# e-c-k-e-r/tortoise-tts

Hardware: AMD Instinct MI355X
Metric: audio-sec/wall-sec (RTF^-1), 16 AR candidates x 80 DDIM steps (higher is better)
Workload: dtype bf16; 1 GPU; configs[1]: 1 utterance/GPU, 64 text tokens, 16 AR candidates x 250 mel tokens (KV-cached decode), latent pass on 16 candidates, 80 DDIM steps with cond-free guidance at T=1088 (11.6 s audio); candidates=16, ddim_steps=80, mel_frames=1088, parallelism=single GPU, small_models=False, vocoder_in_step=False

## Files before the change

### tortoise_tts_amd/csrc/ar.hip

```cpp
#include "ttk_common.h"
#include "ttk_host.h"

using namespace ttk;

namespace {

struct ARLayer {
	float *ln1_g, *ln1_b, *ln2_g, *ln2_b;
	Mat attn, proj, fc, proj2;
};

__global__ void k_build_prefill_emb(const float* cond, int Bc, const int64_t* text, int Tt, int B, int d,
									const float* text_emb, const float* text_pos, const float* mel_emb, const float* mel_pos,
									int start_text, int stop_text, int start_mel, float* out, const int64_t* prompt = nullptr, int prompt_rows = 0, int n_in = 0) {
	const int S = Tt + 4 + n_in;
	const int64_t idx = (int64_t)blockIdx.x * blockDim.x + threadIdx.x;
	const int d4 = d / 4;
	if (idx >= (int64_t)B * S * d4) return;
	const int c = (int)(idx % d4) * 4;
	const int64_t row = idx / d4;
	const int b = (int)(row / S), s = (int)(row - (int64_t)b * S);
	float4 v;
	if (s == 0) {
		v = *(const float4*)(cond + (int64_t)(Bc == 1 ? 0 : b) * d + c);
// ... 16 lines not shown
								   int start_text, int stop_text, int start_mel, int stop_mel, float* out) {
	const int S = Tt + M + 5;
	const int64_t idx = (int64_t)blockIdx.x * blockDim.x + threadIdx.x;
	const int d4 = d / 4;
	if (idx >= (int64_t)B * S * d4) return;
	const int c = (int)(idx % d4) * 4;
	const int64_t row = idx / d4;
	const int b = (int)(row / S), s = (int)(row - (int64_t)b * S);
	float4 v;
	if (s == 0) {
		v = *(const float4*)(cond + (int64_t)b * d + c);
	} else if (s < Tt + 3) {
		const int j = s - 1;
		const int64_t tok = j == 0 ? start_text : (j == Tt + 1 ? stop_text : text[(int64_t)b * Tt + j - 1]);
		const float4 e = *(const float4*)(text_emb + tok * d + c), w = *(const float4*)(text_pos + (int64_t)j * d + c);
		v = make_float4(e.x + w.x, e.y + w.y, e.z + w.z, e.w + w.w);
	} else {
		const int j = s - (Tt + 3);
		const int64_t tok = j == 0 ? start_mel : (j == M + 1 ? stop_mel : codes[(int64_t)b * M + j - 1]);
		const float4 e = *(const float4*)(mel_emb + tok * d + c), w = *(const float4*)(mel_pos + (int64_t)j * d + c);
		v = make_float4(e.x + w.x, e.y + w.y, e.z + w.z, e.w + w.w);
	}
	*(float4*)(out + row * d + c) = v;
}

}

struct ttk_ar {
	ttk_ar_config cfg;
	int dt;
	int wdt;
	size_t es;
	Arena arena;
	std::vector<ARLayer> L;
	float *lnf_g, *lnf_b, *fn_g, *fn_b;
	Mat head;
	float *text_emb, *mel_emb, *mel_pos, *text_pos;
	void *kc, *vc;
	size_t kv_layer_stride;
	int* d_pos;
	int pos_slot = -1;
	int2* d_rowinfo;
	int lines_mode = 0;
	float *x, *qbuf;
	void *attn_out, *hbuf;
	void* x_frag = nullptr;
	int poison = 0;
	int frag_rows = 0;
	int shared_rows = 0;
	int share_prefix = 1;
	const int64_t* rng_args = nullptr; const int64_t* rng_draws = nullptr; float* rng_q = nullptr;
	int* d_health = nullptr;
	float* ring_base = nullptr; const int64_t* ring_idx = nullptr; int64_t ring_stride = 0;
	int64_t* d_ring = nullptr;
	int head_split = 1;
	int lnfold = 1;
	int lean = 1;
	float* slab; int* tickets;
	int wv_proj = 4, wv_proj2 = 8;
	int wv_ln = 4;
	int wv_head = 4;
	int hfrag = 1;
	int narrow2 = 4;
	int narrow = 4;
	int nsplit = 1;
	hipStream_t side[3] = {nullptr, nullptr, nullptr};
	hipEvent_t ev_fork = nullptr, ev_join[3] = {nullptr, nullptr, nullptr};
	WsBuf ws_x, ws_a, ws_qkv, ws_ao, ws_h;
	int B = 0, P = 0, k = 0, ready = 0;
	int Pmax = 0;
	~ttk_ar() {
		for (int i = 0; i < 3; ++i) { if (side[i]) (void)hipStreamDestroy(side[i]); if (ev_join[i]) (void)hipEventDestroy(ev_join[i]); }
		if (ev_fork) (void)hipEventDestroy(ev_fork);
		attn_pos_slot_release(pos_slot);
	}
};

static int poison_scratch(ttk_ar* h, hipStream_t s) {
	if (!h->poison) return TTK_OK;
	for (WsBuf* w : {&h->ws_x, &h->ws_a, &h->ws_qkv, &h->ws_ao, &h->ws_h})
		if (w->p) TTK_HIP(hipMemsetAsync(w->p, 0xFF, w->cap, s));
	return TTK_OK;
}

static int dense_forward(ttk_ar* h, float* x, int B, int S, bool write_kv, hipStream_t s, int kv_row0 = 0, int kv_t0 = 0) {
	const int d = h->cfg.model_dim, H = h->cfg.heads, dt = h->dt;
	const int rows = B * S;
	TTK_TRY(h->ws_a.reserve((size_t)rows * d * h->es));
	TTK_TRY(h->ws_qkv.reserve((size_t)rows * 3 * d * h->es));
	TTK_TRY(h->ws_ao.reserve((size_t)rows * d * h->es));
	TTK_TRY(h->ws_h.reserve((size_t)rows * 4 * d * h->es));
	for (int l = 0; l < h->cfg.layers; ++l) {
		const ARLayer& L = h->L[l];
		launch_layernorm(dt, x, d, rows, d, L.ln1_g, L.ln1_b, nullptr, nullptr, h->ws_a.p, d, 0, s);
		GemmParams g = {};
		g.nseg = 1; g.seg[0] = {h->ws_a.p, d, 0, 0};
		g.W = L.attn.w; g.ldw = L.attn.Kpad; g.M = rows; g.N = 3 * d; g.K = d; g.bias = L.attn.bias;
		g.C = h->ws_qkv.p; g.ldc = 3 * d;
		launch_gemm(dt, g, s);
		if (write_kv) {
			const size_t row0 = (size_t)kv_row0 * H * h->cfg.max_ctx * 64;
			char* kc = (char*)h->kc + ((size_t)l * h->kv_layer_stride + row0) * h->es;
			char* vc = (char*)h->vc + ((size_t)l * h->kv_layer_stride + row0) * h->es;
			launch_kv_scatter(dt, h->ws_qkv.p, B, S, H, kc, vc, h->cfg.max_ctx, s, kv_t0);
		}
		AttnParams a = {};
		a.qkv = h->ws_qkv.p; a.ld = 3 * d; a.q_off = 0; a.k_off = d; a.v_off = 2 * d; a.head_stride = 64;
		a.out = h->ws_ao.p; a.ldo = d; a.nb = B; a.T = S; a.H = H; a.causal = 1; a.bias = nullptr; a.scale = 0.125f;
		launch_attn_fwd(dt, a, s);
		g = {};
		g.nseg = 1; g.seg[0] = {h->ws_ao.p, d, 0, 0};
		g.W = L.proj.w; g.ldw = L.proj.Kpad; g.M = rows; g.N = d; g.K = d; g.bias = L.proj.bias;
		g.residual = x; g.ldr = d; g.C = x; g.ldc = d; g.out_f32 = 1;
		launch_gemm(dt, g, s);
		launch_layernorm(dt, x, d, rows, d, L.ln2_g, L.ln2_b, nullptr, nullptr, h->ws_a.p, d, 0, s);
		g = {};
		g.nseg = 1; g.seg[0] = {h->ws_a.p, d, 0, 0};
		g.W = L.fc.w; g.ldw = L.fc.Kpad; g.M = rows; g.N = 4 * d; g.K = d; g.bias = L.fc.bias; g.act = ACT_GELU_NEW;
		g.C = h->ws_h.p; g.ldc = 4 * d;
		launch_gemm(dt, g, s);
		g = {};
		g.nseg = 1; g.seg[0] = {h->ws_h.p, 4 * d, 0, 0};
		g.W = L.proj2.w; g.ldw = L.proj2.Kpad; g.M = rows; g.N = d; g.K = 4 * d; g.bias = L.proj2.bias;
		g.residual = x; g.ldr = d; g.C = x; g.ldc = d; g.out_f32 = 1;
		launch_gemm(dt, g, s);
	}
	return TTK_OK;
}

static void head_launch(ttk_ar* h, int B, float* logits, float* hidden_out, hipStream_t s) {
	SkinnyParams p = {};
	p.Wp = h->head.wfrag; p.N = h->cfg.number_mel_codes; p.K = h->cfg.model_dim; p.M = B; p.bias = h->head.bias;
	p.ln_count = 2; p.x = h->x; p.ldx = h->cfg.model_dim;
	p.g1 = h->lnf_g; p.b1 = h->lnf_b; p.g2 = h->fn_g; p.b2 = h->fn_b; p.ln_out = hidden_out;
	p.mode = SK_STORE_F32; p.out_f32 = logits; p.ldc = h->cfg.number_mel_codes;
	if (h->rng_q) { p.qbuf = h->rng_q; p.slab = (float*)h->rng_args; p.tickets = (int*)h->rng_draws; }
	launch_skinny(h->dt, p, h->cfg.model_dim >= 1024 ? h->wv_head : 4, s);
}

static void decode_rows(ttk_ar* h, int r0, int nrows, int gi, float* logits_out, float* hidden_out, hipStream_t s, bool bump_pos) {
	const ttk_ar_config& c = h->cfg;
	const int d = c.model_dim, H = c.heads, dt = h->dt;
	const size_t es = h->es;
	float* x = h->x + (size_t)r0 * d;
	float* qbuf = h->qbuf + (size_t)r0 * d;
	char* attn_out = (char*)h->attn_out + (size_t)r0 * d * es;
	char* hbuf = (char*)h->hbuf + (size_t)r0 * 4 * d * es;
	const size_t kv_row = (size_t)H * c.max_ctx * 64 * es;
	const int wv_small = d >= 1024 ? h->wv_ln : 4;
	const int wv_prologue = d >= 1024 ? 8 : 4;
	const bool whole = r0 == 0 && nrows == h->B;
	void* xf = whole ? h->x_frag : nullptr;
	const bool lean = h->lean && whole && h->lnfold && h->hfrag;
	for (int l = 0; l < c.layers; ++l) {
		const ARLayer& L = h->L[l];
		char* kc = (char*)h->kc + (size_t)l * h->kv_layer_stride * es + r0 * kv_row;
		char* vc = (char*)h->vc + (size_t)l * h->kv_layer_stride * es + r0 * kv_row;
		SkinnyParams p = {};
		p.Wp = L.attn.wfrag; p.w8 = L.attn.w8; p.wscale = L.attn.wscale; p.N = 3 * d; p.K = d; p.M = nrows; p.bias = L.attn.bias;
		const bool fold_qkv = h->lnfold && whole && L.attn.wfrag_fold;
		if (fold_qkv) { p.Wp = L.attn.wfrag_fold; p.w8 = 0; p.bias = L.attn.bias_fold; p.g1 = L.attn.csum; p.a = xf; p.lda = d; p.a_frag = 1; }
		else { p.ln_count = 1; p.x = x; p.ldx = d; p.g1 = L.ln1_g; p.b1 = L.ln1_b; }
		p.mode = SK_QKV; p.qbuf = qbuf; p.kcache = kc; p.vcache = vc; p.d_pos = h->d_pos; p.max_ctx = c.max_ctx; p.H = H; p.q_scale = 0.125f;
		GemvParams gq = {};
		gq.Wp = p.Wp; gq.a = xf; gq.bias = p.bias; gq.csum = p.g1; gq.qbuf = qbuf; gq.kcache = kc; gq.vcache = vc; gq.d_pos = h->d_pos;
		gq.M = nrows; gq.N = 3 * d; gq.K = d; gq.max_ctx = c.max_ctx; gq.H = H; gq.q_scale = 0.125f; gq.health = h->d_health;
		if (!(lean && fold_qkv && launch_gemv(dt, GV_QKV, gq, s))) launch_skinny(dt, p, fold_qkv ? wv_small : wv_prologue, s);
		AttnDecodeParams a = {};
		a.qbuf = qbuf; a.kcache = kc; a.vcache = vc; a.d_pos = h->d_pos; a.pos_slot_p1 = h->pos_slot + 1; a.B = nrows; a.H = H; a.max_ctx = c.max_ctx; a.ctx_hint = h->P + 2 + h->k; a.out = attn_out; a.out_frag = h->hfrag && r0 == 0 && nrows == h->B; a.shared_rows = r0 == 0 && h->share_prefix && h->nsplit == 1;
		a.row_info = h->lines_mode && r0 == 0 ? h->d_rowinfo : nullptr;
		launch_attn_decode(dt, a, s);
		p = {};
		p.Wp = L.proj.wfrag; p.w8 = L.proj.w8; p.wscale = L.proj.wscale; p.N = d; p.K = d; p.M = nrows; p.bias = L.proj.bias; p.a = attn_out; p.lda = d; p.a_frag = h->hfrag && r0 == 0 && nrows == h->B;
		p.mode = SK_RESIDUAL; p.out_f32 = x; p.ldc = d; p.narrow = h->narrow; p.out_T = h->lnfold ? xf : nullptr;
		GemvParams gp = {};
		gp.Wp = p.Wp; gp.a = attn_out; gp.bias = p.bias; gp.out_f32 = x; gp.out_T = p.out_T; gp.M = nrows; gp.N = d; gp.K = d; gp.w8 = p.w8; gp.wscale = p.wscale;
		if (!(lean && p.a_frag && h->narrow == 4 && launch_gemv(dt, GV_PROJ, gp, s))) launch_skinny(dt, p, d >= 1024 ? h->wv_proj : 4, s);
		p = {};
		p.Wp = L.fc.wfrag; p.w8 = L.fc.w8; p.wscale = L.fc.wscale; p.N = 4 * d; p.K = d; p.M = nrows; p.bias = L.fc.bias;
		const bool fold_fc = h->lnfold && whole && L.fc.wfrag_fold;
		if (fold_fc) { p.Wp = L.fc.wfrag_fold; p.w8 = 0; p.bias = L.fc.bias_fold; p.g1 = L.fc.csum; p.a = xf; p.lda = d; p.a_frag = 1; }
		else { p.ln_count = 1; p.x = x; p.ldx = d; p.g1 = L.ln2_g; p.b1 = L.ln2_b; }
		p.mode = SK_ACT_T; p.act = ACT_GELU_NEW; p.out_T = hbuf; p.out_frag = h->hfrag && r0 == 0 && nrows == h->B;
		GemvParams gf = {};
		gf.Wp = p.Wp; gf.a = xf; gf.bias = p.bias; gf.csum = p.g1; gf.out_T = hbuf; gf.M = nrows; gf.N = 4 * d; gf.K = d; gf.health = h->d_health;
		if (!(lean && fold_fc && p.out_frag && launch_gemv(dt, GV_FC, gf, s))) launch_skinny(dt, p, fold_fc ? wv_small : wv_prologue, s);
		p = {};
		p.Wp = L.proj2.wfrag; p.w8 = L.proj2.w8; p.wscale = L.proj2.wscale; p.N = d; p.K = 4 * d; p.M = nrows; p.bias = L.proj2.bias; p.a = hbuf; p.lda = 4 * d; p.a_frag = h->hfrag && r0 == 0 && nrows == h->B;
		p.mode = SK_RESIDUAL; p.out_f32 = x; p.ldc = d; p.out_T = h->lnfold ? xf : nullptr;
		p.narrow = h->narrow2;
		if (d >= 1024 && !h->narrow2) {
			p.ksplit = 4; p.slab = h->slab + (size_t)gi * (d / 16) * 4 * 4 * 256; p.tickets = h->tickets + (size_t)gi * (d / 16);
		}
		GemvParams g2 = {};
		g2.Wp = p.Wp; g2.a = hbuf; g2.bias = p.bias; g2.out_f32 = x; g2.out_T = p.out_T; g2.M = nrows; g2.N = d; g2.K = 4 * d; g2.w8 = p.w8; g2.wscale = p.wscale;
		if (!(lean && p.a_frag && h->narrow2 == 4 && launch_gemv(dt, GV_PROJ, g2, s))) launch_skinny(dt, p, d >= 1024 ? h->wv_proj2 : 4, s);
	}
	SkinnyParams p = {};
	p.Wp = h->head.wfrag; p.N = c.number_mel_codes; p.K = d; p.M = nrows; p.bias = h->head.bias;
	p.mode = SK_STORE_F32; p.out_f32 = logits_out + (size_t)r0 * c.number_mel_codes; p.ldc = c.number_mel_codes;
	if (bump_pos) p.d_pos = h->d_pos;
	if (h->rng_q) { p.qbuf = h->rng_q + (size_t)r0 * c.number_mel_codes; p.slab = (float*)h->rng_args; p.tickets = (int*)(h->rng_draws + r0); p.max_ctx = r0; }
	float* hid = hidden_out ? hidden_out + (size_t)r0 * d : nullptr;
	if (h->head_split && whole) {
		if (h->ring_base && !hid) launch_layernorm(dt, x, d, nrows, d, h->lnf_g, h->lnf_b, h->fn_g, h->fn_b, h->attn_out, d, 0, s, 1, nullptr, h->ring_idx, h->ring_stride, h->d_ring);
		else launch_layernorm(dt, x, d, nrows, d, h->lnf_g, h->lnf_b, h->fn_g, h->fn_b, h->attn_out, d, 0, s, 1, hid);
		p.a = h->attn_out; p.lda = d; p.a_frag = 1;
		GemvParams gh = {};
		gh.Wp = p.Wp; gh.a = h->attn_out; gh.bias = p.bias; gh.out_f32 = p.out_f32; gh.d_pos = p.d_pos; gh.noise = p.qbuf; gh.rng = p.slab; gh.draws = (const int64_t*)p.tickets;
		gh.M = nrows; gh.N = c.number_mel_codes; gh.K = d; gh.row0 = r0;
		if (!(lean && launch_gemv(dt, GV_HEAD, gh, s)))
			launch_skinny(dt, p, 4, s);
	} else {
		p.ln_count = 2; p.x = x; p.ldx = d;
		p.g1 = h->lnf_g; p.b1 = h->lnf_b; p.g2 = h->fn_g; p.b2 = h->fn_b; p.ln_out = hid;
		launch_skinny(dt, p, d >= 1024 ? h->wv_head : 4, s);
	}
}

extern "C" {

int ttk_ar_create(ttk_ar** out, const ttk_ar_config* cfg, const ttk_weight_view* w, int n_w) {
	TTK_REQUIRE(out && cfg && w, TTK_E_ARG, "ttk_ar_create: null argument");
	TTK_REQUIRE(cfg->model_dim % 64 == 0 && cfg->heads * 64 == cfg->model_dim, TTK_E_ARG,
				"ttk_ar_create: head_dim must be 64 (model_dim %d, heads %d)", cfg->model_dim, cfg->heads);
	TTK_REQUIRE(cfg->model_dim <= 2048, TTK_E_ARG, "ttk_ar_create: model_dim %d > 2048 unsupported", cfg->model_dim);
	TTK_REQUIRE(cfg->dtype == TTK_F32 || cfg->dtype == TTK_BF16 || cfg->dtype == TTK_F16 || cfg->dtype == TTK_FP8W, TTK_E_ARG, "ttk_ar_create: bad dtype %d", cfg->dtype);
	TTK_REQUIRE(cfg->max_batch >= 1 && cfg->max_batch <= (cfg->dtype == TTK_F32 ? 32 : 64), TTK_E_ARG,
				"ttk_ar_create: max_batch %d out of range", cfg->max_batch);
	TTK_REQUIRE(cfg->max_ctx >= 8, TTK_E_ARG, "ttk_ar_create: max_ctx %d too small", cfg->max_ctx);
	std::unique_ptr<ttk_ar> h(new ttk_ar());
	h->cfg = *cfg;
	h->wdt = cfg->dtype;
	h->dt = kernel_dtype(cfg->dtype);
	h->es = dtype_size(h->dt);
	WeightMap wm(w, n_w);
	const int d = cfg->model_dim;
	h->L.resize(cfg->layers);
	for (int l = 0; l < cfg->layers; ++l) {
		const std::string p = "gpt.h." + std::to_string(l) + ".";
		ARLayer& L = h->L[l];
		TTK_TRY(upload_f32(h->arena, wm, p + "ln_1.weight", d, &L.ln1_g));
		TTK_TRY(upload_f32(h->arena, wm, p + "ln_1.bias", d, &L.ln1_b));
		TTK_TRY(upload_f32(h->arena, wm, p + "ln_2.weight", d, &L.ln2_g));
		TTK_TRY(upload_f32(h->arena, wm, p + "ln_2.bias", d, &L.ln2_b));
		TTK_TRY(upload_mat(h->arena, wm, h->wdt, p + "attn.c_attn.weight", p + "attn.c_attn.bias", PK_KN, 3 * d, d, true, &L.attn));
		TTK_TRY(upload_mat(h->arena, wm, h->wdt, p + "attn.c_proj.weight", p + "attn.c_proj.bias", PK_KN, d, d, true, &L.proj));
		TTK_TRY(upload_mat(h->arena, wm, h->wdt, p + "mlp.c_fc.weight", p + "mlp.c_fc.bias", PK_KN, 4 * d, d, true, &L.fc));
		TTK_TRY(upload_mat(h->arena, wm, h->wdt, p + "mlp.c_proj.weight", p + "mlp.c_proj.bias", PK_KN, d, 4 * d, true, &L.proj2));
		{
			TTK_TRY(fold_layernorm(h->arena, wm, h->dt, p + "attn.c_attn.weight", p + "attn.c_attn.bias", p + "ln_1.weight", p + "ln_1.bias", &L.attn));
			TTK_TRY(fold_layernorm(h->arena, wm, h->dt, p + "mlp.c_fc.weight", p + "mlp.c_fc.bias", p + "ln_2.weight", p + "ln_2.bias", &L.fc));
		}
	}
	TTK_TRY(upload_f32(h->arena, wm, "gpt.ln_f.weight", d, &h->lnf_g));
	TTK_TRY(upload_f32(h->arena, wm, "gpt.ln_f.bias", d, &h->lnf_b));
	TTK_TRY(upload_f32(h->arena, wm, "final_norm.weight", d, &h->fn_g));
	TTK_TRY(upload_f32(h->arena, wm, "final_norm.bias", d, &h->fn_b));
	TTK_TRY(upload_mat(h->arena, wm, h->dt, "mel_head.weight", "mel_head.bias", PK_NK, cfg->number_mel_codes, d, true, &h->head));
	TTK_TRY(upload_f32(h->arena, wm, "text_embedding.weight", (int64_t)cfg->number_text_tokens_p1 * d, &h->text_emb));
	TTK_TRY(upload_f32(h->arena, wm, "mel_embedding.weight", (int64_t)cfg->number_mel_codes * d, &h->mel_emb));
	TTK_TRY(upload_f32(h->arena, wm, "mel_pos_embedding.emb.weight", (int64_t)cfg->max_mel_seq_len * d, &h->mel_pos));
	TTK_TRY(upload_f32(h->arena, wm, "text_pos_embedding.emb.weight", (int64_t)cfg->max_text_seq_len * d, &h->text_pos));
	h->kv_layer_stride = (size_t)cfg->max_batch * cfg->heads * cfg->max_ctx * 64;
	TTK_TRY(h->arena.alloc(&h->kc, h->kv_layer_stride * cfg->layers * h->es));
	TTK_TRY(h->arena.alloc(&h->vc, h->kv_layer_stride * cfg->layers * h->es));
	TTK_TRY(h->arena.alloc((void**)&h->d_pos, (size_t)(4 + 2 * cfg->max_batch) * sizeof(int)));
	h->d_rowinfo = (int2*)(h->d_pos + 4);
	h->d_health = h->d_pos + 2;
	if (hipMemset(h->d_pos, 0, (size_t)(4 + 2 * cfg->max_batch) * sizeof(int)) != hipSuccess) return TTK_E_HIP;
	{
		int* words = nullptr;
		h->pos_slot = attn_pos_slot_acquire(&words);
		if (h->pos_slot >= 0) {
			h->d_pos = words;
			if (hipMemset(h->d_pos, 0, 2 * sizeof(int)) != hipSuccess) return TTK_E_HIP;
		}
	}
	TTK_TRY(h->arena.alloc((void**)&h->d_ring, sizeof(int64_t)));
	if (hipMemset(h->d_ring, 0, sizeof(int64_t)) != hipSuccess) return TTK_E_HIP;
	TTK_TRY(h->arena.alloc((void**)&h->x, (size_t)cfg->max_batch * d * sizeof(float)));
	TTK_TRY(h->arena.alloc((void**)&h->qbuf, (size_t)cfg->max_batch * d * sizeof(float)));
	const size_t frag_rows = (size_t)16 * decode_row_tiles(cfg->max_batch);
	h->frag_rows = (int)frag_rows;
	for (int B = 1; B <= cfg->max_batch; ++B)
		if (16 * decode_row_tiles(B) > h->frag_rows) { set_error("ttk_ar_create: %d rows would request %d fragment rows, %d allocated", B, 16 * decode_row_tiles(B), h->frag_rows); return TTK_E_STATE; }
	TTK_TRY(h->arena.alloc(&h->attn_out, frag_rows * d * h->es));
	if (hipMemset(h->attn_out, 0, frag_rows * d * h->es) != hipSuccess) return TTK_E_HIP;
	TTK_TRY(h->arena.alloc(&h->hbuf, frag_rows * 4 * d * h->es));
	if (hipMemset(h->hbuf, 0, frag_rows * 4 * d * h->es) != hipSuccess) return TTK_E_HIP;
	TTK_TRY(h->arena.alloc(&h->x_frag, frag_rows * d * h->es));
	if (hipMemset(h->x_frag, 0, frag_rows * d * h->es) != hipSuccess) return TTK_E_HIP;
	TTK_TRY(h->arena.alloc((void**)&h->slab, (size_t)4 * (d / 16) * 4 * 4 * 256 * sizeof(float)));
	TTK_TRY(h->arena.alloc((void**)&h->tickets, (size_t)4 * (d / 16) * sizeof(int)));
	if (hipMemset(h->tickets, 0, (size_t)4 * (d / 16) * sizeof(int)) != hipSuccess) return TTK_E_HIP;
	{
		const char* ep = getenv("TTK_DEBUG_POISON");
		h->poison = ep && atoi(ep) != 0;
		const char* en = getenv("TTK_AR_NARROW");
		h->narrow = en ? atoi(en) : 4;
		const char* ef = getenv("TTK_AR_HFRAG");
		h->hfrag = ef ? (atoi(ef) != 0) : 1;
		const char* en2 = getenv("TTK_AR_NARROW2");
		h->narrow2 = en2 ? atoi(en2) : h->narrow;
		const char* e1 = getenv("TTK_AR_WV_PROJ");
		const char* e2 = getenv("TTK_AR_WV_PROJ2");
		if (e1 && atoi(e1) >= 4 && atoi(e1) <= 16) h->wv_proj = atoi(e1);
		if (h->dt == DT_F32) { h->wv_proj = 8; h->wv_ln = 8; h->wv_proj2 = 8; }
		if (e2 && atoi(e2) >= 4 && atoi(e2) <= 16) h->wv_proj2 = atoi(e2);
		const char* e4 = getenv("TTK_AR_WV_LN");
		if (e4 && atoi(e4) >= 4 && atoi(e4) <= 16) h->wv_ln = atoi(e4);
		const char* e3 = getenv("TTK_AR_WV_HEAD");
		if (e3 && (atoi(e3) == 4 || atoi(e3) == 8)) h->wv_head = atoi(e3);
		const char* es = getenv("TTK_AR_SHARE_PREFIX");
		h->share_prefix = es ? (atoi(es) != 0) : 1;
		const char* eh = getenv("TTK_AR_HEAD_SPLIT");
		h->head_split = eh ? (atoi(eh) != 0) : 1;
		const char* el = getenv("TTK_AR_LNFOLD");
		h->lnfold = el ? (atoi(el) != 0) : 1;
		const char* eg = getenv("TTK_AR_LEAN");
		h->lean = eg ? (atoi(eg) != 0) : 1;
		const char* e = getenv("TTK_AR_SPLIT");
		h->nsplit = e ? atoi(e) : 1;
		if (h->nsplit != 1 && h->nsplit != 2 && h->nsplit != 4) h->nsplit = 1;
		if (hipEventCreateWithFlags(&h->ev_fork, hipEventDisableTiming) != hipSuccess) return TTK_E_HIP;
		for (int i = 0; i < 3; ++i) {
			if (hipStreamCreateWithFlags(&h->side[i], hipStreamNonBlocking) != hipSuccess) return TTK_E_HIP;
			if (hipEventCreateWithFlags(&h->ev_join[i], hipEventDisableTiming) != hipSuccess) return TTK_E_HIP;
		}
	}
	hipError_t e = hipDeviceSynchronize();
	if (e != hipSuccess) { set_error("ttk_ar_create: %s", hipGetErrorString(e)); return TTK_E_HIP; }
	*out = h.release();
	return TTK_OK;
}

int ttk_ar_destroy(ttk_ar* h) {
	if (!h) return TTK_OK;
	(void)hipDeviceSynchronize();
	delete h;
	return TTK_OK;
}

static int prefill_impl(ttk_ar* h, const float* cond_latent, int Bc, const int64_t* text, int Tt, const int64_t* prompt, int prompt_rows, int n_in, int B, float* logits_out,
						void* stream, const char* who) {
	TTK_REQUIRE(h && cond_latent && text && logits_out, TTK_E_ARG, "%s: null argument", who);
	const ttk_ar_config& c = h->cfg;
	TTK_REQUIRE(B >= 1 && B <= c.max_batch, TTK_E_ARG, "%s: B=%d exceeds max_batch=%d", who, B, c.max_batch);
	TTK_REQUIRE(Bc == 1 || Bc == B, TTK_E_ARG, "%s: cond batch %d must be 1 or B=%d", who, Bc, B);
	TTK_REQUIRE(Tt >= 1 && Tt + 2 <= c.max_text_seq_len, TTK_E_ARG, "%s: %d text tokens exceed the position table (%d)", who, Tt, c.max_text_seq_len - 2);
	TTK_REQUIRE(n_in == 0 || (prompt && (prompt_rows == 1 || prompt_rows == B)), TTK_E_ARG, "%s: %d prompt tokens need 1 or B=%d prompt rows (got %d)", who, n_in, B, prompt_rows);
	TTK_REQUIRE(n_in >= 0 && n_in + 2 < c.max_mel_seq_len, TTK_E_ARG, "%s: %d prompt tokens exceed the mel position table (%d)", who, n_in, c.max_mel_seq_len);
	const int S = Tt + 4 + n_in, d = c.model_dim;
	TTK_REQUIRE(S + 1 <= c.max_ctx, TTK_E_ARG, "%s: prefix of %d rows does not fit max_ctx=%d", who, S, c.max_ctx);
	hipStream_t s = (hipStream_t)stream;
	const bool shared = Bc == 1 && B > 1 && h->share_prefix && h->nsplit == 1 && (n_in == 0 || prompt_rows == 1);
	const int Bp = shared ? 1 : B;
	TTK_TRY(h->ws_x.reserve((size_t)Bp * S * d * sizeof(float)));
	float* x = (float*)h->ws_x.p;
	const int64_t total = (int64_t)Bp * S * (d / 4);
	hipLaunchKernelGGL(k_build_prefill_emb, dim3((unsigned)((total + 255) / 256)), dim3(256), 0, s, cond_latent, Bc, text, Tt, Bp, d,
					   h->text_emb, h->text_pos, h->mel_emb, h->mel_pos, c.start_text_token, c.stop_text_token, c.start_mel_token, x, prompt, prompt_rows, n_in);
	TTK_TRY(dense_forward(h, x, Bp, S, true, s));
	launch_copy_rows(x + (size_t)(S - 1) * d, shared ? 0 : (int64_t)S * d, h->x, d, B, d, s);
	head_launch(h, B, logits_out, nullptr, s);
	launch_set_int(h->d_pos, S, s);
	launch_set_int(h->d_pos + 1, shared ? S : 0, s);
	TTK_TRY(poison_scratch(h, s));
	h->B = B; h->P = h->Pmax = Tt + 3; h->k = n_in; h->ready = 1; h->lines_mode = 0;
	h->shared_rows = shared ? S : 0;
	TTK_HIP(hipGetLastError());
	return TTK_OK;
}

int ttk_ar_prefill(ttk_ar* h, const float* cond_latent, int Bc, const int64_t* text, int Tt, int B, float* logits_out, void* stream) {
	return prefill_impl(h, cond_latent, Bc, text, Tt, nullptr, 0, 0, B, logits_out, stream, "ttk_ar_prefill");
}

int ttk_ar_prefill_prompted(ttk_ar* h, const float* cond_latent, int Bc, const int64_t* text, int Tt, const int64_t* prompt, int prompt_rows, int n_prompt, int B,
							float* logits_out, void* stream) {
	TTK_REQUIRE(n_prompt >= 1 && prompt, TTK_E_ARG, "ttk_ar_prefill_prompted: needs at least one prompt token");
	return prefill_impl(h, cond_latent, Bc, text, Tt, prompt, prompt_rows, n_prompt, B, logits_out, stream, "ttk_ar_prefill_prompted");
}

int ttk_ar_prefill_lines(ttk_ar* h, const float* cond_latents, const int64_t* text, const int* text_len, int n_lines, int rows_per_line,
						 float* logits_out, void* stream) {
	TTK_REQUIRE(h && cond_latents && text && text_len && logits_out, TTK_E_ARG, "ttk_ar_prefill_lines: null argument");
	const ttk_ar_config& c = h->cfg;
	const int B = n_lines * rows_per_line, d = c.model_dim;
	TTK_REQUIRE(n_lines >= 1 && rows_per_line >= 1 && B <= c.max_batch, TTK_E_ARG, "ttk_ar_prefill_lines: %d lines x %d candidates exceed max_batch=%d", n_lines, rows_per_line, c.max_batch);
	TTK_REQUIRE(h->share_prefix && h->nsplit == 1, TTK_E_STATE, "ttk_ar_prefill_lines: needs the shared-prefix decode (TTK_AR_SHARE_PREFIX=1, TTK_AR_SPLIT=1)");
	int Smax = 0;
	for (int g = 0; g < n_lines; ++g) {
		const int Tt = text_len[g];
		TTK_REQUIRE(Tt >= 1 && Tt + 2 <= c.max_text_seq_len, TTK_E_ARG, "ttk_ar_prefill_lines: line %d: %d text tokens exceed the position table (%d)", g, Tt, c.max_text_seq_len - 2);
		TTK_REQUIRE(Tt + 5 <= c.max_ctx, TTK_E_ARG, "ttk_ar_prefill_lines: line %d: prefix of %d rows does not fit max_ctx=%d", g, Tt + 4, c.max_ctx);
		Smax = Tt + 4 > Smax ? Tt + 4 : Smax;
	}
	hipStream_t s = (hipStream_t)stream;
	TTK_TRY(h->ws_x.reserve((size_t)Smax * d * sizeof(float)));
	float* x = (float*)h->ws_x.p;
	int64_t toff = 0;
	for (int g = 0; g < n_lines; ++g) {
		const int Tt = text_len[g], S = Tt + 4, r0 = g * rows_per_line, start = Smax - S;
		const int64_t total = (int64_t)S * (d / 4);
		hipLaunchKernelGGL(k_build_prefill_emb, dim3((unsigned)((total + 255) / 256)), dim3(256), 0, s, cond_latents + (size_t)g * d, 1, text + toff, Tt, 1, d,
						   h->text_emb, h->text_pos, h->mel_emb, h->mel_pos, c.start_text_token, c.stop_text_token, c.start_mel_token, x);
		TTK_TRY(dense_forward(h, x, 1, S, true, s, r0, start));
		launch_copy_rows(x + (size_t)(S - 1) * d, 0, h->x + (size_t)r0 * d, d, rows_per_line, d, s);
		launch_fill_int2((int*)(h->d_rowinfo + r0), start, r0, rows_per_line, s);
		toff += Tt;
	}
	head_launch(h, B, logits_out, nullptr, s);
	launch_set_int(h->d_pos, Smax, s);
	launch_set_int(h->d_pos + 1, Smax, s);
	TTK_TRY(poison_scratch(h, s));
	h->B = B; h->P = h->Pmax = Smax - 1; h->k = 0; h->ready = 1; h->lines_mode = 1;
	h->shared_rows = Smax;
	TTK_HIP(hipGetLastError());
	return TTK_OK;
}

static int decode_impl(ttk_ar* h, const int64_t* tok, float* logits_out, float* hidden_out, void* stream, const char* who) {
	TTK_REQUIRE(h && logits_out, TTK_E_ARG, "%s: null argument", who);
	TTK_REQUIRE(h->ready, TTK_E_STATE, "%s: call ttk_ar_prefill first", who);
	const ttk_ar_config& c = h->cfg;
	const int B = h->B, d = c.model_dim;
	TTK_REQUIRE(h->Pmax + 1 + h->k + 1 <= c.max_ctx, TTK_E_STATE, "%s: KV cache full (max_ctx=%d)", who, c.max_ctx);
	TTK_REQUIRE(B <= c.max_batch && 16 * decode_row_tiles(B) <= h->frag_rows, TTK_E_STATE, "%s: %d rows request %d fragment rows, the handle holds %d (max_batch=%d)", who, B,
				16 * decode_row_tiles(B), h->frag_rows, c.max_batch);
	TTK_REQUIRE((h->lnfold && h->nsplit == 1) || B <= 32, TTK_E_STATE, "%s: the LayerNorm-prologue decode kernels (TTK_AR_LNFOLD=0 / TTK_AR_SPLIT) hold at most 32 candidates' rows in LDS; B=%d", who, B);
	TTK_REQUIRE(h->k + 2 < c.max_mel_seq_len, TTK_E_STATE, "%s: mel position table exhausted (%d rows)", who, c.max_mel_seq_len);
	TTK_REQUIRE(!h->ring_base || (h->head_split && h->nsplit == 1), TTK_E_STATE, "%s: the hidden ring needs the default decode form (TTK_AR_HEAD_SPLIT=1, TTK_AR_SPLIT=1)", who);
	hipStream_t s = (hipStream_t)stream;
	if (tok) launch_decode_embed(h->mel_emb, tok, h->mel_pos, h->d_pos, 1 - h->P, c.max_mel_seq_len, h->x, B, d, s, h->lnfold ? h->x_frag : nullptr, elem_kind(h->dt));
	int nsplit = h->nsplit;
	while (nsplit > 1 && B / nsplit < 1) nsplit >>= 1;
	if (nsplit > 1) {
		TTK_HIP(hipEventRecord(h->ev_fork, s));
		for (int gi = 1; gi < nsplit; ++gi) TTK_HIP(hipStreamWaitEvent(h->side[gi - 1], h->ev_fork, 0));
	}
	for (int gi = 0; gi < nsplit; ++gi) {
		hipStream_t gs = gi == 0 ? s : h->side[gi - 1];
		const int r0 = (B * gi) / nsplit, r1 = (B * (gi + 1)) / nsplit;
		decode_rows(h, r0, r1 - r0, gi, logits_out, hidden_out, gs, nsplit == 1);
	}
	for (int gi = 1; gi < nsplit; ++gi) {
		TTK_HIP(hipEventRecord(h->ev_join[gi - 1], h->side[gi - 1]));
		TTK_HIP(hipStreamWaitEvent(s, h->ev_join[gi - 1], 0));
	}
	if (nsplit > 1) launch_add_int(h->d_pos, 1, s);
	h->k += 1;
	TTK_HIP(hipGetLastError());
	return TTK_OK;
}

int ttk_ar_decode(ttk_ar* h, const int64_t* tok, float* logits_out, float* hidden_out, void* stream) {
	TTK_REQUIRE(tok, TTK_E_ARG, "ttk_ar_decode: null argument");
	return decode_impl(h, tok, logits_out, hidden_out, stream, "ttk_ar_decode");
}

int ttk_ar_decode_next(ttk_ar* h, float* logits_out, float* hidden_out, void* stream) {
	return decode_impl(h, nullptr, logits_out, hidden_out, stream, "ttk_ar_decode_next");
}

int ttk_ar_sample_next(ttk_ar* h, const ttk_sample_args* a, void* stream) {
	TTK_REQUIRE(h && a, TTK_E_ARG, "ttk_ar_sample_next: null argument");
	TTK_REQUIRE(h->ready, TTK_E_STATE, "ttk_ar_sample_next: call ttk_ar_prefill first");
	TTK_REQUIRE(a->B == h->B && a->V == h->cfg.number_mel_codes, TTK_E_ARG, "ttk_ar_sample_next: shape (B %d, V %d) is not the prefilled one (B %d, V %d)",
				a->B, a->V, h->B, h->cfg.number_mel_codes);
	return launch_sample_step(a, h->mel_emb, h->mel_pos, h->x, h->cfg.model_dim, h->cfg.max_mel_seq_len, h->lnfold ? h->x_frag : nullptr, elem_kind(h->dt),
							  (hipStream_t)stream, "ttk_ar_sample_next");
}

// ... 81 lines not shown
```

### tortoise_tts_amd/csrc/gemv.hip

```cpp
#include <hip/hip_ext.h>

#include "ttk_common.h"
#include "ttk_kernels.h"
#include "ttk_rng.h"

namespace ttk {

#ifndef TTK_NT
#define TTK_NT 1
#endif
#if TTK_NT
#define GV_WLOAD(p) __builtin_nontemporal_load(p)
#else
#define GV_WLOAD(p) (*(p))
#endif

#if defined(TTK_STAMPS) && TTK_STAMPS == 2
#define GV_STAMP(i) do { if (p.stamps && (threadIdx.x & 63) == 0) { unsigned long long* st_ = p.stamps + ((size_t)blockIdx.x * 16 + (threadIdx.x >> 6)) * 8; \
	st_[(i)] = __builtin_amdgcn_s_memrealtime(); if ((i) == 0) st_[7] = __builtin_amdgcn_s_getreg(20 | (0 << 6) | (3 << 11)); } } while (0)
#define GV_STAMPD(i, dep) do { if (p.stamps) { unsigned tmp_; unsigned long long t_; \
	asm volatile("s_nop 7\n\tv_readfirstlane_b32 %0, %2\n\ts_memrealtime %1\n\ts_waitcnt lgkmcnt(0)" : "=s"(tmp_), "=s"(t_) : "v"(dep) : "memory"); \
	if ((threadIdx.x & 63) == 0) p.stamps[((size_t)blockIdx.x * 16 + (threadIdx.x >> 6)) * 8 + (i)] = t_; } } while (0)
#else
#define GV_STAMP(i) do {} while (0)
#define GV_STAMPD(i, dep) do {} while (0)
#endif

template <typename T, bool W8> struct GvW {
	typedef typename Frag<T>::type raw;
	static __device__ __forceinline__ typename Frag<T>::type dec(raw r) { return r; }
};
template <> struct GvW<bf16, true> {
	typedef unsigned raw __attribute__((ext_vector_type(2)));
	static __device__ __forceinline__ bf16x8 dec(raw r) {
		typedef float f2 __attribute__((ext_vector_type(2)));
		const f2 a = __builtin_amdgcn_cvt_pk_f32_fp8((int)r[0], false), b = __builtin_amdgcn_cvt_pk_f32_fp8((int)r[0], true);
		const f2 c = __builtin_amdgcn_cvt_pk_f32_fp8((int)r[1], false), d = __builtin_amdgcn_cvt_pk_f32_fp8((int)r[1], true);
		return bf16x8{(bf16)a[0], (bf16)a[1], (bf16)b[0], (bf16)b[1], (bf16)c[0], (bf16)c[1], (bf16)d[0], (bf16)d[1]};
	}
};

template <typename T> __device__ __forceinline__ void fold_stats(const typename Frag<T>::type& a, float& s1, float& s2) {
#pragma unroll
	for (int j = 0; j < 8; ++j) { const float f = (float)a[j]; s1 += f; s2 = fmaf(f, f, s2); }
}
template <> __device__ __forceinline__ void fold_stats<bf16>(const bf16x8& a, float& s1, float& s2) {
	typedef __bf16 bf16x2 __attribute__((ext_vector_type(2)));
	const bf16x2 one = {(bf16)1.0f, (bf16)1.0f};
#pragma unroll
	for (int j = 0; j < 8; j += 2) {
		const bf16x2 x = {a[j], a[j + 1]};
		s2 = __builtin_amdgcn_fdot2_f32_bf16(x, x, s2, false);
		s1 = __builtin_amdgcn_fdot2_f32_bf16(x, one, s1, false);
	}
}
template <> __device__ __forceinline__ void fold_stats<f16>(const f16x8& a, float& s1, float& s2) {
	typedef _Float16 f16x2 __attribute__((ext_vector_type(2)));
	const f16x2 one = {(f16)1.0f, (f16)1.0f};
#pragma unroll
	for (int j = 0; j < 8; j += 2) {
		const f16x2 x = {a[j], a[j + 1]};
		s2 = __builtin_amdgcn_fdot2(x, x, s2, false);
		s1 = __builtin_amdgcn_fdot2(x, one, s1, false);
	}
}

template <typename T, int MT, int ROLE, int NW, int KPW, bool W8>
__global__ __launch_bounds__(64 * NW) void k_gemv(GemvParams p) {
	typedef typename Frag<T>::type FragT;
	typedef GvW<T, W8> WF;
	typedef typename WF::raw WRaw;
	constexpr int ES = sizeof(T);
	constexpr bool FOLD = ROLE == GV_QKV || ROLE == GV_FC;
	constexpr bool NARROW = ROLE == GV_PROJ;
	constexpr int KS = NW * KPW;
	extern __shared__ __attribute__((aligned(16))) float gv_red[];
	float* red = gv_red;
	float* rstat = red + NW * MT * 64 * 4;
	asm volatile("" :: "s"(p.Wp), "s"(p.a), "s"(p.bias), "s"(p.csum), "s"(p.out_f32), "s"(p.out_T), "s"(p.qbuf), "s"(p.kcache), "s"(p.vcache),
				 "s"(p.d_pos), "s"(p.noise), "s"(p.rng), "s"(p.draws), "s"(p.health), "s"(p.M), "s"(p.N), "s"(p.max_ctx), "s"(p.H), "s"(p.row0), "s"(p.q_scale), "s"(p.wscale));
	GV_STAMP(0);
	const int tid = threadIdx.x, lane = tid & 63, wave = tid >> 6;
	int nt, sub = 0;
	if (NARROW) { const int b = blockIdx.x; nt = ((b >> 5) << 3) + (b & 7); sub = (b >> 3) & 3; }
	else nt = blockIdx.x;

	const int l2 = lane, r = wave & 3;
	const int n = NARROW ? nt * 16 + 4 * sub + (l2 & 3) : nt * 16 + (l2 & 15);
	const bool mine = tid < 256 && (!NARROW || (l2 & 15) < 4) && n < p.N;
	const int nn = n < p.N ? n : p.N - 1;
	float bias = 0.f, fcs = 0.f, res[MT];
	RngArgs rng = {};
	int64_t draw[MT];
	int kv_pos = 0;
	if (ROLE == GV_QKV) kv_pos = *p.d_pos;
	if (ROLE == GV_HEAD && p.d_pos && blockIdx.x == 0 && tid == 0) *(int*)p.d_pos += 1;
	const bool noise = ROLE == GV_HEAD && p.noise != nullptr;
	if (p.bias) bias = p.bias[nn];
	if (FOLD) fcs = p.csum[nn];
	if (noise) rng = *(const RngArgs*)p.rng;
#pragma unroll
	for (int mt = 0; mt < MT; ++mt) {
		res[mt] = 0.f; draw[mt] = 0;
		int m = mt * 16 + 4 * (l2 >> 4) + r;
		m = m < p.M ? m : p.M - 1;
		if (ROLE == GV_PROJ) res[mt] = p.out_f32[(int64_t)m * p.N + nn];
		if (noise) draw[mt] = p.draws[m];
	}

	constexpr int OPREGS = (MT + 1) * (ES == 4 ? 8 : 4);
	constexpr int PRE0 = 64 / OPREGS >= 8 ? 8 : (64 / OPREGS >= 4 ? 4 : (64 / OPREGS >= 2 ? 2 : 1));
	constexpr int PRE = PRE0 < KPW ? PRE0 : KPW;
	static_assert(KPW % PRE == 0, "k-steps per wave must be a multiple of the operand batch");
	const int ks0 = wave * KPW;
	const WRaw* wp = (const WRaw*)p.Wp + ((int64_t)nt * KS + ks0) * 64 + (NARROW ? ((lane & ~15) | (4 * sub + (lane & 3))) : lane);
	const FragT* ap = (const FragT*)p.a + (int64_t)ks0 * 64 + lane;
	f32x4 acc[MT];
	float fs1[MT], fs2[MT];
#pragma unroll
	for (int mt = 0; mt < MT; ++mt) { acc[mt] = f32x4{0.f, 0.f, 0.f, 0.f}; fs1[mt] = 0.f; fs2[mt] = 0.f; }
	constexpr bool WLDS = NARROW && ES == 2;
	if constexpr (WLDS) {
		static_assert(KPW % 4 == 0, "dense weight requests cover four k-steps");
		constexpr int WL = KPW / 4;
		WRaw* wl = (WRaw*)(rstat) + wave * (KPW * 16);
		const WRaw* wd = (const WRaw*)p.Wp + ((int64_t)nt * KS + ks0 + (lane >> 4)) * 64 + ((lane >> 2) & 3) * 16 + 4 * sub + (lane & 3);
		WRaw wq[WL];
#pragma unroll
		for (int i = 0; i < WL; ++i) wq[i] = GV_WLOAD(wd + i * 4 * 64);
		FragT a0[PRE][MT];
#pragma unroll
		for (int u = 0; u < PRE; ++u)
#pragma unroll
			for (int mt = 0; mt < MT; ++mt) a0[u][mt] = ap[((int64_t)mt * KS + u) * 64];
		GV_STAMP(2);
		__builtin_amdgcn_sched_barrier(0);
#pragma unroll
		for (int i = 0; i < WL; ++i) wl[i * 64 + lane] = wq[i];
		const int rd = ((lane >> 4) << 2) + (lane & 3);
#pragma unroll
		for (int kb = 0; kb < KPW; kb += PRE) {
			FragT a[PRE][MT];
			if (kb + PRE < KPW) {
#pragma unroll
				for (int u = 0; u < PRE; ++u)
#pragma unroll
					for (int mt = 0; mt < MT; ++mt) a[u][mt] = ap[((int64_t)mt * KS + kb + PRE + u) * 64];
			}
			__builtin_amdgcn_sched_barrier(0);
#pragma unroll
			for (int u = 0; u < PRE; ++u) {
				const WRaw b = wl[(kb + u) * 16 + rd];
#pragma unroll
				for (int mt = 0; mt < MT; ++mt) acc[mt] = mma16<T>(a0[u][mt], WF::dec(b), acc[mt]);
			}
			if (kb + PRE < KPW) {
#pragma unroll
				for (int u = 0; u < PRE; ++u)
#pragma unroll
					for (int mt = 0; mt < MT; ++mt) a0[u][mt] = a[u][mt];
			}
		}
	} else {
#pragma unroll
	for (int kb = 0; kb < KPW; kb += PRE) {
		WRaw b[PRE];
		FragT a[PRE][MT];
#pragma unroll
		for (int u = 0; u < PRE; ++u) {
			b[u] = GV_WLOAD(wp + (kb + u) * 64);
#pragma unroll
			for (int mt = 0; mt < MT; ++mt) a[u][mt] = ap[((int64_t)mt * KS + kb + u) * 64];
		}
		if (kb == 0) GV_STAMP(2);
		__builtin_amdgcn_sched_barrier(0);
#pragma unroll
		for (int u = 0; u < PRE; ++u)
#pragma unroll
			for (int mt = 0; mt < MT; ++mt) {
				if (FOLD) fold_stats<T>(a[u][mt], fs1[mt], fs2[mt]);
				acc[mt] = mma16<T>(a[u][mt], WF::dec(b[u]), acc[mt]);
			}
	}
	}
	if (FOLD) {
#pragma unroll
		for (int mt = 0; mt < MT; ++mt) {
			fs1[mt] = fold16_add(fs1[mt]); fs2[mt] = fold16_add(fs2[mt]);
			fs1[mt] = fold32_add(fs1[mt]); fs2[mt] = fold32_add(fs2[mt]);
			if (lane < 16) *(float2*)(rstat + ((wave * MT + mt) * 16 + lane) * 2) = make_float2(fs1[mt], fs2[mt]);
		}
	}
	GV_STAMPD(3, acc[0][0]);
#pragma unroll
	for (int mt = 0; mt < MT; ++mt) *(f32x4*)(red + ((wave * MT + mt) * 64 + lane) * 4) = acc[mt];
	__syncthreads();
	GV_STAMP(4);
	if (!mine) return;
#pragma unroll
	for (int mt = 0; mt < MT; ++mt) {
		const int m = mt * 16 + 4 * (l2 >> 4) + r;
		if (m >= p.M) continue;
		float vs = 0.f;
#pragma unroll
		for (int w = 0; w < NW; ++w) vs += red[((w * MT + mt) * 64 + l2) * 4 + r];
		float v;
		if (FOLD) {
			float a1 = 0.f, a2 = 0.f;
#pragma unroll
			for (int w = 0; w < NW; ++w) { const float2 t = *(const float2*)(rstat + ((w * MT + mt) * 16 + 4 * (l2 >> 4) + r) * 2); a1 += t.x; a2 += t.y; }
			const float mean = a1 / (float)(32 * KS);
			const float var = fmaxf(fmaf(-mean, mean, a2 / (float)(32 * KS)), 0.f);
			const float rstd = rsqrtf(var + 1e-5f);
			v = (vs - mean * fcs) * rstd + bias;
			if (p.health && blockIdx.x == 0 && (l2 & 15) == 0) {
				const int bad = (mean * mean > 64.f * (var + 1e-5f) ? 1 : 0) | (a2 - a2 != 0.f ? 2 : 0);
				if (bad) atomicOr(p.health, bad);
			}
		} else {
			v = (W8 ? vs * p.wscale : vs) + bias;
		}
		if (ROLE == GV_HEAD) {
			p.out_f32[(int64_t)m * p.N + n] = v;
			if (noise) {
				int mrow = p.row0 + m;
				const int grp = (int)rng.group;
				if (grp > 0) while (mrow >= grp) mrow -= grp;
				p.noise[(int64_t)m * p.N + n] = torch_exponential_at(rng, draw[mt], (rng.row0 + mrow) * (int64_t)p.N + n);
			}
		} else if (ROLE == GV_PROJ) {
			p.out_f32[(int64_t)m * p.N + n] = res[mt] + v;
			if (p.out_T) ((T*)p.out_T)[((((int64_t)mt * (p.N >> 5) + (n >> 5)) * 64 + ((n >> 3) & 3) * 16 + (m & 15)) * 8 + (n & 7))] = cvt<T>(res[mt] + v);
		} else if (ROLE == GV_FC) {
			((T*)p.out_T)[((((int64_t)mt * (p.N >> 5) + (n >> 5)) * 64 + ((n >> 3) & 3) * 16 + (m & 15)) * 8 + (n & 7))] = cvt<T>(gelu_new_f(v));
		} else {
			constexpr int d = 32 * KS;
			const int which = n / d, c = n - which * d;
			if (which == 0) {
				p.qbuf[(int64_t)m * d + c] = v * p.q_scale;
			} else {
				const int h = c >> 6, dd = c & 63;
				T* cache = (T*)(which == 1 ? p.kcache : p.vcache);
				if (kv_pos < p.max_ctx) cache[(((int64_t)m * p.H + h) * p.max_ctx + kv_pos) * 64 + dd] = cvt<T>(v);
			}
		}
	}
	GV_STAMP(5);
#if defined(TTK_STAMPS) && TTK_STAMPS == 2
	asm volatile("s_waitcnt vmcnt(0)" ::: "memory");
	GV_STAMP(6);
#endif
}

template <typename T, int MT, int ROLE, int NW, int KPW, bool W8>
static void gemv_go(const GemvParams& p, hipStream_t s, hipEvent_t ea, hipEvent_t eb) {
	constexpr bool FOLD = ROLE == GV_QKV || ROLE == GV_FC;
	const int tiles = (p.N + 15) / 16;
	const int grid = ROLE == GV_PROJ ? tiles * 4 : tiles;
	const size_t lds = (size_t)NW * MT * 64 * 4 * sizeof(float) + (FOLD ? (size_t)NW * MT * 16 * 2 * sizeof(float) : 0)
					   + (ROLE == GV_PROJ && sizeof(T) == 2 ? (size_t)NW * KPW * 16 * (W8 ? 8 : 16) : 0);
	hipExtLaunchKernelGGL((k_gemv<T, MT, ROLE, NW, KPW, W8>), dim3(grid), dim3(64 * NW), (unsigned)lds, s, ea, eb, 0, p);
}

template <typename T, int ROLE, int NW, int KPW, bool W8>
static void gemv_mt(const GemvParams& p, hipStream_t s, hipEvent_t ea, hipEvent_t eb) {
	const int mt = decode_row_tiles(p.M);
	if (mt == 1) gemv_go<T, 1, ROLE, NW, KPW, W8>(p, s, ea, eb);
	else if (mt == 2) gemv_go<T, 2, ROLE, NW, KPW, W8>(p, s, ea, eb);
	else if (mt == 3 && sizeof(T) == 2) gemv_go<T, sizeof(T) == 2 ? 3 : 2, ROLE, NW, KPW, W8>(p, s, ea, eb);
	else if (sizeof(T) == 2) gemv_go<T, sizeof(T) == 2 ? 4 : 2, ROLE, NW, KPW, W8>(p, s, ea, eb);
}

template <typename T, int ROLE, bool W8>
static bool gemv_role(const GemvParams& p, hipStream_t s, hipEvent_t ea, hipEvent_t eb) {
	constexpr bool F32 = sizeof(T) == 4;
	if (ROLE == GV_HEAD) {
		if (p.K != 1024) return false;
		gemv_mt<T, ROLE, 4, 8, W8>(p, s, ea, eb);
	} else if (p.K == 1024) {
		gemv_mt<T, ROLE, F32 ? 8 : 4, F32 ? 4 : 8, W8>(p, s, ea, eb);
	} else if (p.K == 4096 && ROLE == GV_PROJ) {
		gemv_mt<T, ROLE, 8, 16, W8>(p, s, ea, eb);
	} else {
		return false;
	}
	return true;
}

bool gemv_supported(int dt, int role, const GemvParams& p) {
	if (dt != DT_BF16 && dt != DT_F16 && dt != DT_F32) return false;
	if (p.M < 1 || p.M > (dt == DT_F32 ? 32 : 64)) return false;
	if (p.w8 && (dt != DT_BF16 || role != GV_PROJ)) return false;
	if (role == GV_HEAD) return p.K == 1024;
	if (role == GV_PROJ) return (p.K == 1024 || p.K == 4096) && p.N % 128 == 0;
	if (role == GV_QKV) return p.K == 1024 && p.N == 3 * p.K;
	return p.K == 1024 && p.N % 32 == 0;
}

bool launch_gemv(int dt, int role, const GemvParams& p, hipStream_t s) {
	if (!gemv_supported(dt, role, p)) return false;
	hipEvent_t ea = nullptr, eb = nullptr;
	if (g_prof_on) prof_pair(PROF_SKINNY, (double)p.N * p.K * (p.w8 ? 1 : dtype_size(dt)) + 4.0 * p.N + 4.0 * p.M * p.K + 4.0 * p.M * p.N, &ea, &eb);
#define GV_DISPATCH(T, W8) \
	(role == GV_QKV ? gemv_role<T, GV_QKV, false>(p, s, ea, eb) : role == GV_FC ? gemv_role<T, GV_FC, false>(p, s, ea, eb) : \
	 role == GV_HEAD ? gemv_role<T, GV_HEAD, false>(p, s, ea, eb) : gemv_role<T, GV_PROJ, W8>(p, s, ea, eb))
	if (dt == DT_BF16) return p.w8 ? GV_DISPATCH(bf16, true) : GV_DISPATCH(bf16, false);
	if (dt == DT_F16) return GV_DISPATCH(f16, false);
	return GV_DISPATCH(float, false);
#undef GV_DISPATCH
}

}
```

Baseline: 40.62 audio-sec/wall-sec.

## Prefetch gemv operand blocks further ahead and add lean=2 proj fallback

Restructures the k_gemv inner loop so activation fragments (and, in the non-LDS path, weight fragments) are held in a full KPW-sized register array and loaded one or more blocks ahead of the MFMA consumption. This applies to QKV/FC roles and the narrow LDS-weight path. The goal is to hide global-load latency behind matrix math. It also adds a TTK_AR_LEAN=2 mode that sends the proj/proj2 GEMMs back to the skinny kernel, and makes the role dispatch if-constexpr so the K=4096 instantiation is only built for proj. The cost is higher register pressure, which may reduce occupancy or cause spills.

```diff
diff --git a/tortoise_tts_amd/csrc/ar.hip b/tortoise_tts_amd/csrc/ar.hip
--- a/tortoise_tts_amd/csrc/ar.hip
+++ b/tortoise_tts_amd/csrc/ar.hip
@@ -192,6 +192,7 @@
 	const bool whole = r0 == 0 && nrows == h->B;
 	void* xf = whole ? h->x_frag : nullptr;
 	const bool lean = h->lean && whole && h->lnfold && h->hfrag;
+	const bool lean_proj = lean && h->lean != 2;
 	for (int l = 0; l < c.layers; ++l) {
 		const ARLayer& L = h->L[l];
 		char* kc = (char*)h->kc + (size_t)l * h->kv_layer_stride * es + r0 * kv_row;
@@ -215,7 +216,7 @@
 		p.mode = SK_RESIDUAL; p.out_f32 = x; p.ldc = d; p.narrow = h->narrow; p.out_T = h->lnfold ? xf : nullptr;
 		GemvParams gp = {};
 		gp.Wp = p.Wp; gp.a = attn_out; gp.bias = p.bias; gp.out_f32 = x; gp.out_T = p.out_T; gp.M = nrows; gp.N = d; gp.K = d; gp.w8 = p.w8; gp.wscale = p.wscale;
-		if (!(lean && p.a_frag && h->narrow == 4 && launch_gemv(dt, GV_PROJ, gp, s))) launch_skinny(dt, p, d >= 1024 ? h->wv_proj : 4, s);
+		if (!(lean_proj && p.a_frag && h->narrow == 4 && launch_gemv(dt, GV_PROJ, gp, s))) launch_skinny(dt, p, d >= 1024 ? h->wv_proj : 4, s);
 		p = {};
 		p.Wp = L.fc.wfrag; p.w8 = L.fc.w8; p.wscale = L.fc.wscale; p.N = 4 * d; p.K = d; p.M = nrows; p.bias = L.fc.bias;
 		const bool fold_fc = h->lnfold && whole && L.fc.wfrag_fold;
@@ -234,7 +235,7 @@
 		}
 		GemvParams g2 = {};
 		g2.Wp = p.Wp; g2.a = hbuf; g2.bias = p.bias; g2.out_f32 = x; g2.out_T = p.out_T; g2.M = nrows; g2.N = d; g2.K = 4 * d; g2.w8 = p.w8; g2.wscale = p.wscale;
-		if (!(lean && p.a_frag && h->narrow2 == 4 && launch_gemv(dt, GV_PROJ, g2, s))) launch_skinny(dt, p, d >= 1024 ? h->wv_proj2 : 4, s);
+		if (!(lean_proj && p.a_frag && h->narrow2 == 4 && launch_gemv(dt, GV_PROJ, g2, s))) launch_skinny(dt, p, d >= 1024 ? h->wv_proj2 : 4, s);
 	}
 	SkinnyParams p = {};
 	p.Wp = h->head.wfrag; p.N = c.number_mel_codes; p.K = d; p.M = nrows; p.bias = h->head.bias;
@@ -359,7 +360,7 @@
 		const char* el = getenv("TTK_AR_LNFOLD");
 		h->lnfold = el ? (atoi(el) != 0) : 1;
 		const char* eg = getenv("TTK_AR_LEAN");
-		h->lean = eg ? (atoi(eg) != 0) : 1;
+		h->lean = eg ? atoi(eg) : 1;
 		const char* e = getenv("TTK_AR_SPLIT");
 		h->nsplit = e ? atoi(e) : 1;
 		if (h->nsplit != 1 && h->nsplit != 2 && h->nsplit != 4) h->nsplit = 1;
diff --git a/tortoise_tts_amd/csrc/gemv.hip b/tortoise_tts_amd/csrc/gemv.hip
--- a/tortoise_tts_amd/csrc/gemv.hip
+++ b/tortoise_tts_amd/csrc/gemv.hip
@@ -64,6 +64,8 @@
 		s1 = __builtin_amdgcn_fdot2(x, one, s1, false);
 	}
 }
+
+constexpr bool gv_ahead_ok(int es, int mt, int role) { return (role == GV_QKV || role == GV_FC) && !(es == 2 && mt == 3); }
 
 template <typename T, int MT, int ROLE, int NW, int KPW, bool W8>
 __global__ __launch_bounds__(64 * NW) void k_gemv(GemvParams p) {
@@ -108,6 +110,9 @@
 		if (noise) draw[mt] = p.draws[m];
 	}
 
+#ifndef TTK_GEMV_AHEAD
+#define TTK_GEMV_AHEAD 1
+#endif
 	constexpr int OPREGS = (MT + 1) * (ES == 4 ? 8 : 4);
 	constexpr int PRE0 = 64 / OPREGS >= 8 ? 8 : (64 / OPREGS >= 4 ? 4 : (64 / OPREGS >= 2 ? 2 : 1));
 	constexpr int PRE = PRE0 < KPW ? PRE0 : KPW;
@@ -119,69 +124,80 @@
 	float fs1[MT], fs2[MT];
 #pragma unroll
 	for (int mt = 0; mt < MT; ++mt) { acc[mt] = f32x4{0.f, 0.f, 0.f, 0.f}; fs1[mt] = 0.f; fs2[mt] = 0.f; }
+	FragT a[KPW][MT];
 	constexpr bool WLDS = NARROW && ES == 2;
 	if constexpr (WLDS) {
 		static_assert(KPW % 4 == 0, "dense weight requests cover four k-steps");
 		constexpr int WL = KPW / 4;
+		constexpr bool AHEAD = TTK_GEMV_AHEAD != 0;
+		constexpr int G = !AHEAD ? PRE : (MT == 1 ? KPW : (PRE >= 2 ? PRE / 2 : 1));
+		constexpr int NB = KPW / G;
+		constexpr int WIN = MT == 2 && KPW == 8 ? 2 * PRE - G : 2 * PRE;
+		constexpr int LOOK0 = !AHEAD ? 1 : WIN / G - 1;
+		constexpr int LOOK = LOOK0 < NB - 1 ? LOOK0 : NB - 1;
+		constexpr int UP = AHEAD ? LOOK + 1 : 1;
 		WRaw* wl = (WRaw*)(rstat) + wave * (KPW * 16);
 		const WRaw* wd = (const WRaw*)p.Wp + ((int64_t)nt * KS + ks0 + (lane >> 4)) * 64 + ((lane >> 2) & 3) * 16 + 4 * sub + (lane & 3);
 		WRaw wq[WL];
 #pragma unroll
 		for (int i = 0; i < WL; ++i) wq[i] = GV_WLOAD(wd + i * 4 * 64);
-		FragT a0[PRE][MT];
-#pragma unroll
-		for (int u = 0; u < PRE; ++u)
-#pragma unroll
-			for (int mt = 0; mt < MT; ++mt) a0[u][mt] = ap[((int64_t)mt * KS + u) * 64];
+#pragma unroll
+		for (int k = 0; k < UP * G; ++k)
+#pragma unroll
+			for (int mt = 0; mt < MT; ++mt) a[k][mt] = ap[((int64_t)mt * KS + k) * 64];
 		GV_STAMP(2);
 		__builtin_amdgcn_sched_barrier(0);
 #pragma unroll
 		for (int i = 0; i < WL; ++i) wl[i * 64 + lane] = wq[i];
 		const int rd = ((lane >> 4) << 2) + (lane & 3);
 #pragma unroll
-		for (int kb = 0; kb < KPW; kb += PRE) {
-			FragT a[PRE][MT];
-			if (kb + PRE < KPW) {
-#pragma unroll
-				for (int u = 0; u < PRE; ++u)
-#pragma unroll
-					for (int mt = 0; mt < MT; ++mt) a[u][mt] = ap[((int64_t)mt * KS + kb + PRE + u) * 64];
+		for (int bi = 0; bi < NB; ++bi) {
+			if (bi + LOOK >= UP && bi + LOOK < NB) {
+#pragma unroll
+				for (int u = 0; u < G; ++u)
+#pragma unroll
+					for (int mt = 0; mt < MT; ++mt) a[(bi + LOOK) * G + u][mt] = ap[((int64_t)mt * KS + (bi + LOOK) * G + u) * 64];
 			}
 			__builtin_amdgcn_sched_barrier(0);
 #pragma unroll
-			for (int u = 0; u < PRE; ++u) {
-				const WRaw b = wl[(kb + u) * 16 + rd];
-#pragma unroll
-				for (int mt = 0; mt < MT; ++mt) acc[mt] = mma16<T>(a0[u][mt], WF::dec(b), acc[mt]);
-			}
-			if (kb + PRE < KPW) {
-#pragma unroll
-				for (int u = 0; u < PRE; ++u)
-#pragma unroll
-					for (int mt = 0; mt < MT; ++mt) a0[u][mt] = a[u][mt];
+			for (int u = 0; u < G; ++u) {
+				const WRaw b = wl[(bi * G + u) * 16 + rd];
+#pragma unroll
+				for (int mt = 0; mt < MT; ++mt) acc[mt] = mma16<T>(a[bi * G + u][mt], WF::dec(b), acc[mt]);
 			}
 		}
 	} else {
-#pragma unroll
-	for (int kb = 0; kb < KPW; kb += PRE) {
-		WRaw b[PRE];
-		FragT a[PRE][MT];
-#pragma unroll
-		for (int u = 0; u < PRE; ++u) {
-			b[u] = GV_WLOAD(wp + (kb + u) * 64);
-#pragma unroll
-			for (int mt = 0; mt < MT; ++mt) a[u][mt] = ap[((int64_t)mt * KS + kb + u) * 64];
-		}
-		if (kb == 0) GV_STAMP(2);
-		__builtin_amdgcn_sched_barrier(0);
-#pragma unroll
-		for (int u = 0; u < PRE; ++u)
-#pragma unroll
-			for (int mt = 0; mt < MT; ++mt) {
-				if (FOLD) fold_stats<T>(a[u][mt], fs1[mt], fs2[mt]);
-				acc[mt] = mma16<T>(a[u][mt], WF::dec(b[u]), acc[mt]);
-			}
-	}
+		constexpr int NB = KPW / PRE;
+		constexpr bool AHEAD = TTK_GEMV_AHEAD != 0 && NB > 1 && gv_ahead_ok(ES, MT, ROLE);
+		constexpr int LOOK = AHEAD ? 1 : 0;
+		WRaw b[KPW];
+#pragma unroll
+		for (int k = 0; k < (LOOK + 1) * PRE; ++k) {
+			b[k] = GV_WLOAD(wp + k * 64);
+#pragma unroll
+			for (int mt = 0; mt < MT; ++mt) a[k][mt] = ap[((int64_t)mt * KS + k) * 64];
+		}
+		GV_STAMP(2);
+#pragma unroll
+		for (int bi = 0; bi < NB; ++bi) {
+			if (bi >= 1 && bi + LOOK < NB) {
+#pragma unroll
+				for (int u = 0; u < PRE; ++u) {
+					const int k = (bi + LOOK) * PRE + u;
+					b[k] = GV_WLOAD(wp + k * 64);
+#pragma unroll
+					for (int mt = 0; mt < MT; ++mt) a[k][mt] = ap[((int64_t)mt * KS + k) * 64];
+				}
+			}
+			__builtin_amdgcn_sched_barrier(0);
+#pragma unroll
+			for (int u = 0; u < PRE; ++u)
+#pragma unroll
+				for (int mt = 0; mt < MT; ++mt) {
+					if (FOLD) fold_stats<T>(a[bi * PRE + u][mt], fs1[mt], fs2[mt]);
+					acc[mt] = mma16<T>(a[bi * PRE + u][mt], WF::dec(b[bi * PRE + u]), acc[mt]);
+				}
+		}
 	}
 	if (FOLD) {
 #pragma unroll
@@ -274,15 +290,18 @@
 template <typename T, int ROLE, bool W8>
 static bool gemv_role(const GemvParams& p, hipStream_t s, hipEvent_t ea, hipEvent_t eb) {
 	constexpr bool F32 = sizeof(T) == 4;
-	if (ROLE == GV_HEAD) {
+	if constexpr (ROLE == GV_HEAD) {
 		if (p.K != 1024) return false;
 		gemv_mt<T, ROLE, 4, 8, W8>(p, s, ea, eb);
-	} else if (p.K == 1024) {
-		gemv_mt<T, ROLE, F32 ? 8 : 4, F32 ? 4 : 8, W8>(p, s, ea, eb);
-	} else if (p.K == 4096 && ROLE == GV_PROJ) {
-		gemv_mt<T, ROLE, 8, 16, W8>(p, s, ea, eb);
 	} else {
-		return false;
+		if (p.K == 1024) {
+			gemv_mt<T, ROLE, F32 ? 8 : 4, F32 ? 4 : 8, W8>(p, s, ea, eb);
+		} else if constexpr (ROLE == GV_PROJ) {
+			if (p.K != 4096) return false;
+			gemv_mt<T, ROLE, 8, 16, W8>(p, s, ea, eb);
+		} else {
+			return false;
+		}
 	}
 	return true;
 }
```

New measurement: 40.55 audio-sec/wall-sec. Within noise of the previous version (-0.2%).
